# otiliastr/coper

Hardware: AMD Instinct MI355X
Metric: scored triples/sec (1-vs-all) (higher is better)
Workload: dtype fp16x3 (fp32 values split into two fp16 terms, 3 fp16 MFMAs per product, fp32 accumulate; comparisons closer than the split's error decided by the fp32 chain)

## Files before the change

### coper_amd/csrc/kernels_dense_fused_bf16.hip

```cpp
#include "bf16x3_chain.h"
#include "coper_internal.h"
#ifdef COPER_DBG_GROUP_CLK
#include <hip/hip_runtime.h>
__device__ unsigned long long g_group_clk[8];
extern "C" __attribute__((visibility("default"))) int coper_dbg_group_clock(unsigned long long* out) {
  return hipMemcpyFromSymbol(out, HIP_SYMBOL(g_group_clk), sizeof(unsigned long long) * 8) == hipSuccess ? 0 : 1;
}
#define GROUP_CLK(i) do { __syncthreads(); if (threadIdx.x == 0) g_group_clk[i] = wall_clock64(); } while (0)
#endif
#include "group_body.h"
#include "conv_fold.h"

namespace coper {

typedef float f32x4 __attribute__((ext_vector_type(4)));
typedef unsigned u32x4 __attribute__((ext_vector_type(4)));

#define MFMA16_BF16(a, b, c) S16_MFMA16(a, b, c)
#define MFMA16_X3(ahi, alo, bhi, blo, c) \
  { (c) = MFMA16_BF16(alo, bhi, c); (c) = MFMA16_BF16(ahi, blo, c); (c) = MFMA16_BF16(ahi, bhi, c); }


#ifndef COPER_FUSED_PMAX
#define COPER_FUSED_PMAX 3
#endif
#ifndef COPER_FUSED_PBUDGET
#define COPER_FUSED_PBUDGET 220
#endif


#define FW_DECL u32x4 W[P][NW][2]
#define FW_HI(s_, j_) W[s_][j_][0]
#define FW_LO(s_, j_) W[s_][j_][1]
#define FW_LO_RAW(s_, j_) W[s_][j_][1]
#define FW_PRE(s_)
#define FW_WREG3 (3 * NW * 8)

struct FusedConvArgs {
  const float* e1_rows;
  const int32_t* sorted_row;
  const int32_t* sorted_rid;
  const float* ent;
  const float* rel_emb;
  const float* conv_w;
  const float* conv_b;
  const float* scale;
  const float* shift;
  int per_rel_conv, d, r, in_w, in_hw, Wo, img_stride, x_exp;
  int img_exp;
  int64_t* chk;
  int w_div, w_rem;
  int32_t* bad;
};

#ifdef COPER_DBG_FUSED_CLOCK
__device__ unsigned long long g_fused_ph[8 * 2048];
extern "C" __attribute__((visibility("default"))) int coper_dbg_fused_phases(unsigned long long* out, int n) {
  return hipMemcpyFromSymbol(out, HIP_SYMBOL(g_fused_ph), sizeof(unsigned long long) * 8 * (n < 2048 ? n : 2048)) == hipSuccess ? 0 : 1;
}
#define FUSED_PH(i_)                                                                                            \
  do {                                                                                                          \
    const int w_ = blockIdx.x + gridDim.x * (blockIdx.y + gridDim.y * blockIdx.z);                              \
    if ((threadIdx.x & 63) == 0 && w_ < 2048) g_fused_ph[8 * w_ + (i_)] = __builtin_amdgcn_s_memrealtime();     \
  } while (0)
#else
#define FUSED_PH(i_) do { } while (0)
#endif
struct FusedFinConst {
  const int32_t* perm; const float* fc_b; const float* scale; const float* shift; const int32_t* w_exp; float* x3m;
  int per_rel_bias, x_exp, d, pad;
};
struct FusedFin {
  float* h_out; const FusedFinConst* c;
};
constexpr int FUSED_STAGE_WGS = 16;


__device__ __forceinline__ void fused_load_images(unsigned* __restrict__ img, const FusedConvArgs& A, int start, int n,
                                                  int t0, int t1) {
  const int wave = __builtin_amdgcn_readfirstlane(threadIdx.x >> 6), lane = threadIdx.x & 63;
  const int q0 = wave * 16;
  if (q0 < n) {
    int qi = q0 + (lane & 15);
    if (qi > n - 1) qi = n - 1;
    int my_row = A.sorted_row[start + qi], my_rid = A.sorted_rid[start + qi];
#ifdef COPER_DBG_NO_GROUP_CHK
    const bool chk = false;
#else
    const bool chk = A.chk != nullptr && (blockIdx.y | blockIdx.z) == 0;
#endif
    int64_t live_rel = 0, live_e1 = 0;
    const int chk_row = my_row, chk_rid = my_rid;
    if (chk) group_chk_issue(A.chk, start + qi, live_rel, live_e1);
#ifdef COPER_DBG_FUSED_NO_IMG
    my_row = -1;
#endif
    const float* base = A.e1_rows ? A.e1_rows : A.ent;
    const int len = t1 - t0, PD = (A.img_stride - 1) >> 1, eI = A.img_exp;
    auto fetch2 = [&](const int row, const int rid, const int t) -> float2 {
      if (t >= t1) return make_float2(0.f, 0.f);
      if (t < A.d) return row >= 0 ? *(const float2*)(base + (int64_t)row * A.d + t) : make_float2(0.f, 0.f);
      return *(const float2*)(A.rel_emb + (int64_t)rid * A.r + (t - A.d));
    };
    auto put2 = [&](const int q, const int pp, const float2 x) {
      unsigned short h0, l0, h1, l1;
      split1_s16(x3_scale(x.x, eI), h0, l0);
      split1_s16(x3_scale(x.y, eI), h1, l1);
      img[q * A.img_stride + pp] = (unsigned)h0 | ((unsigned)h1 << 16);
      img[q * A.img_stride + PD + pp] = (unsigned)l0 | ((unsigned)l1 << 16);
    };
    float2 v[16][2];
#pragma unroll
    for (int u = 0; u < 16; ++u) {
      const int row = __builtin_amdgcn_readlane(my_row, u), rid = __builtin_amdgcn_readlane(my_rid, u);
#pragma unroll
      for (int h = 0; h < 2; ++h) v[u][h] = fetch2(row, rid, t0 + 2 * (lane + 64 * h));
    }
#pragma unroll
    for (int u = 0; u < 16; ++u)
      if (q0 + u < n) {
#pragma unroll
        for (int h = 0; h < 2; ++h)
          if (2 * (lane + 64 * h) < len) put2(q0 + u, lane + 64 * h, v[u][h]);
        if (lane == 0) img[(q0 + u) * A.img_stride + 2 * PD] = 0u;
      }
    if (len > 256) {
      for (int u = 0; u < 16 && q0 + u < n; ++u) {
        const int row = __builtin_amdgcn_readlane(my_row, u), rid = __builtin_amdgcn_readlane(my_rid, u);
        for (int pp = 128 + lane; 2 * pp < len; pp += 64) put2(q0 + u, pp, fetch2(row, rid, t0 + 2 * pp));
      }
    }
    if (chk) group_chk_verdict(A.chk, live_rel, live_e1, chk_row, chk_rid);
  }
  asm volatile("s_waitcnt lgkmcnt(0)" ::: "memory");
  __builtin_amdgcn_s_barrier();
}

typedef unsigned fused_img_t;
template <int NFB, int NB, bool WNT>
__device__ __forceinline__ void fused_matrix_role(const uint4* __restrict__ xring, fused_img_t* __restrict__ img,
                                                  const uint4* __restrict__ Whi, const uint4* __restrict__ Wlo,
                                                  const FusedConvArgs& A, int64_t relw, int64_t relw_w, int start, int n, int fb0,
                                                  int nfb, int64_t ks32n, int64_t kb, int64_t ke, int t0, int t1,
                                                  float* __restrict__ zdst, int d_pad16, int wave, const FusedFin& Fn, int64_t ks32s) {
  constexpr int NFULL = NFB / 4;
  constexpr int REM = NFB % 4 ? 1 : 0;
  static_assert(NFB % 4 <= 1, "at most one left-over feature block");
  constexpr int NRQ = REM ? (NB + 3) / 4 : 0;
  constexpr int NW = NFULL + REM;
  constexpr int P = (COPER_FUSED_PMAX >= 3 && (NFULL * NB + NRQ) * 4 + FW_WREG3 + 44 <= COPER_FUSED_PBUDGET) ? 3 : 2;
  constexpr int XSTAGE = 2 * NB * 64;
  const int lane = threadIdx.x & 63;
  const int nk = (int)(ke - kb);
  const uint4* wp[NW][2];
#pragma unroll
  for (int j = 0; j < NW; ++j) {
    int fb = fb0 + (j < NFULL ? wave + 4 * j : 4 * NFULL);
    if (fb > nfb - 1) fb = nfb - 1;
    int64_t o = ((relw_w * nfb + fb) * ks32s + kb) * 64;
    wp[j][0] = Whi + o;
    wp[j][1] = (const uint4*)(Wlo + o);
  }
  FW_DECL;
#define FUSED_W_LOAD(p_) (WNT ? __builtin_nontemporal_load(p_) : *(p_))
#define W_ISSUE(s, kk)                                                                                 \
  {                                                                                                    \
    _Pragma("unroll") for (int j = 0; j < NW; ++j) {                                                   \
      FW_HI(s, j) = FUSED_W_LOAD((const u32x4*)(wp[j][0] + (int64_t)(kk)*64) + lane);                 \
      FW_LO_RAW(s, j) = FUSED_W_LOAD((const u32x4*)((const uint4*)wp[j][1] + (int64_t)(kk)*64) + lane); \
    }                                                                                                  \
  }
#pragma unroll
  for (int t = 0; t < P; ++t)
    if (t < nk) W_ISSUE(t, t);
  if (wave == 0) FUSED_PH(0);
  fused_load_images(img, A, start, n, t0, t1);
  if (wave == 0) FUSED_PH(1);
  f32x4 acc[NFULL][NB], accr[NRQ > 0 ? NRQ : 1];
#pragma unroll
  for (int j = 0; j < NFULL; ++j)
#pragma unroll
    for (int q = 0; q < NB; ++q) acc[j][q] = (f32x4){0.f, 0.f, 0.f, 0.f};
#pragma unroll
  for (int t = 0; t < NRQ; ++t) accr[t] = (f32x4){0.f, 0.f, 0.f, 0.f};
#ifdef COPER_DBG_FUSED_NO_MFMA
#define M_STEP(s2)                                                                                  \
  {                                                                                                 \
    __builtin_amdgcn_s_barrier();                                                                   \
    const uint4* xb = xring + ((s2)&1) * XSTAGE + lane;                                             \
    _Pragma("unroll") for (int j = 0; j < NW; ++j) {                                                \
      acc[0][0][0] += __uint_as_float(FW_HI((s2) % P, j)[0] ^ FW_LO_RAW((s2) % P, j)[1]);           \
      acc[0][0][1] += __uint_as_float(FW_HI((s2) % P, j)[2] ^ FW_LO_RAW((s2) % P, j)[0]);           \
    }                                                                                               \
    acc[0][0][2] += __uint_as_float(xb[0].x);                                                       \
  }
#else
#ifdef COPER_DBG_FUSED_NO_XREAD
#define M_LD(i_) make_uint4((unsigned)lane, (unsigned)(i_), 0x3c003c00u, 0x3c003c00u)
#else
#define M_LD(i_) xb[i_]
#endif
#ifndef COPER_FUSED_XPF
#define COPER_FUSED_XPF 2
#endif
#ifndef COPER_FUSED_XBUDGET
#define COPER_FUSED_XBUDGET 220
#endif
  constexpr int NV = NB + (NRQ > 0 ? 1 : 0);
  constexpr int XPF = (P == 3 && (NFULL * NB + NRQ) * 4 + FW_WREG3 + 44 > COPER_FUSED_XBUDGET) ? 1 : COPER_FUSED_XPF, XR = XPF + 1;
  const int qr = wave < NB ? wave : NB - 1;
#define M_LDV_H(v_) M_LD(((v_) < NB ? (v_) : qr) * 64)
#define M_LDV_L(v_) M_LD((NB + ((v_) < NB ? (v_) : qr)) * 64)
#define M_STEP(s2)                                                                                  \
  {                                                                                                 \
    FW_PRE((s2) % P)                                                                                \
    __builtin_amdgcn_s_barrier();                                                                   \
    const uint4* xb = xring + ((s2)&1) * XSTAGE + lane;                                             \
    uint4 bhq[XR], blq[XR];                                                                         \
    _Pragma("unroll") for (int v = 0; v < XPF && v < NV; ++v) { bhq[v] = M_LDV_H(v); blq[v] = M_LDV_L(v); } \
    __builtin_amdgcn_sched_group_barrier(0x100, 2 * (XPF < NV ? XPF : NV), 0);                      \
    _Pragma("unroll") for (int q = 0; q < NB; ++q) {                                                \
      if (q + XPF < NV) {                                                                           \
        bhq[(q + XPF) % XR] = M_LDV_H(q + XPF); blq[(q + XPF) % XR] = M_LDV_L(q + XPF);             \
        __builtin_amdgcn_sched_group_barrier(0x100, 2, 0);                                          \
      }                                                                                             \
      __builtin_amdgcn_sched_group_barrier(0x008, 3 * NFULL, 0);                                    \
      const uint4 bh = bhq[q % XR], bl = blq[q % XR];                                               \
      _Pragma("unroll") for (int j = 0; j < NFULL; ++j)                                             \
          acc[j][q] = MFMA16_BF16(FW_LO((s2) % P, j), bh, acc[j][q]);                               \
      _Pragma("unroll") for (int j = 0; j < NFULL; ++j)                                             \
          acc[j][q] = MFMA16_BF16(FW_HI((s2) % P, j), bl, acc[j][q]);                               \
      _Pragma("unroll") for (int j = 0; j < NFULL; ++j)                                             \
          acc[j][q] = MFMA16_BF16(FW_HI((s2) % P, j), bh, acc[j][q]);                               \
    }                                                                                               \
    _Pragma("unroll") for (int t = 0; t < NRQ; ++t) {                                               \
      const int q = wave + 4 * t < NB ? wave + 4 * t : NB - 1;  \
      uint4 bh, bl;                                                                                 \
      if (t == 0) { bh = bhq[NB % XR]; bl = blq[NB % XR]; }     \
      else { bh = M_LD(q * 64); bl = M_LD((NB + q) * 64); }                                         \
      accr[t] = MFMA16_BF16(FW_LO((s2) % P, NFULL), bh, accr[t]);                                   \
      accr[t] = MFMA16_BF16(FW_HI((s2) % P, NFULL), bl, accr[t]);                                   \
      accr[t] = MFMA16_BF16(FW_HI((s2) % P, NFULL), bh, accr[t]);                                   \
    }                                                                                               \
  }
#endif
  int k0 = 0;
  for (; k0 + 2 * P <= nk; k0 += 2 * P) {
#pragma unroll
    for (int s2 = 0; s2 < 2 * P; ++s2) {
      M_STEP(s2);
#ifndef COPER_DBG_FUSED_NO_W
      const int kn = k0 + s2 + P;
      W_ISSUE(s2 % P, kn < nk ? kn : 0);
#endif
    }
    if (k0 == 0 && wave == 0) FUSED_PH(2);
  }
#pragma unroll
  for (int s2 = 0; s2 < 2 * P - 1; ++s2) {
    if (k0 + s2 < nk) {
      M_STEP(s2);
#ifndef COPER_DBG_FUSED_NO_W
      if (k0 + s2 + P < nk) W_ISSUE(s2 % P, k0 + s2 + P);
#endif
    }
  }
#undef M_STEP
#undef W_ISSUE
  if (wave == 0) FUSED_PH(3);
#ifdef COPER_DBG_FUSED_NO_STORE
  if (acc[0][0][0] != 1.2345f) return;
#endif
  if (Fn.h_out) {
    const FusedFinConst Fc = *Fn.c;
    const int d = Fc.d;
    const int zexp = -((Fc.w_exp ? Fc.w_exp[Fc.per_rel_bias ? relw : 0] : 0) + Fc.x_exp);
    const float* bsrc = Fc.per_rel_bias ? Fc.fc_b + relw * d : Fc.fc_b;
    float m = 0.f;
    int qrow[NB];
#pragma unroll
    for (int q = 0; q < NB; ++q) {
      const int qi = q * 16 + (lane & 15);
      qrow[q] = qi < n ? Fc.perm[start + qi] : -1;
    }
    auto fin = [&](const f32x4& a, const int fb, const int q, const float4& b4, const float4& s4, const float4& t4) {
      const int k0 = fb * 16 + 4 * (lane >> 4);
      if (fb >= nfb || qrow[q] < 0 || k0 >= d) return;
      float z0 = 0.f, z1 = 0.f, z2 = 0.f, z3 = 0.f;
      z0 += a[0]; z1 += a[1]; z2 += a[2]; z3 += a[3];
      float4 v;
      v.x = fmaxf(fmaf(x3_scale(z0, zexp) + b4.x, s4.x, t4.x), 0.f);
      v.y = fmaxf(fmaf(x3_scale(z1, zexp) + b4.y, s4.y, t4.y), 0.f);
      v.z = fmaxf(fmaf(x3_scale(z2, zexp) + b4.z, s4.z, t4.z), 0.f);
      v.w = fmaxf(fmaf(x3_scale(z3, zexp) + b4.w, s4.w, t4.w), 0.f);
      m = fmaxf(m, fmaxf(fmaxf(v.x, v.y), fmaxf(v.z, v.w)));
      *(float4*)(Fn.h_out + (int64_t)qrow[q] * d + k0) = v;
    };
    auto quad = [&](const float* p, const int fb) -> float4 {
      const int k0 = fb * 16 + 4 * (lane >> 4);
      return (fb < nfb && k0 < d) ? *(const float4*)(p + k0) : make_float4(0.f, 0.f, 0.f, 0.f);
    };
#pragma unroll
    for (int j = 0; j < NFULL; ++j) {
      const int fb = fb0 + wave + 4 * j;
      const float4 b4 = quad(bsrc, fb), s4 = quad(Fc.scale, fb), t4 = quad(Fc.shift, fb);
#pragma unroll
      for (int q = 0; q < NB; ++q) fin(acc[j][q], fb, q, b4, s4, t4);
    }
    if (NRQ > 0) {
      const int fb = fb0 + 4 * NFULL;
      const float4 b4 = quad(bsrc, fb), s4 = quad(Fc.scale, fb), t4 = quad(Fc.shift, fb);
#pragma unroll
      for (int t = 0; t < NRQ; ++t) {
        const int q = wave + 4 * t;
        if (q < NB) {
          const int qi = q * 16 + (lane & 15);
          const int row = qi < n ? Fc.perm[start + qi] : -1;
          const int k0 = fb * 16 + 4 * (lane >> 4);
          if (fb < nfb && row >= 0 && k0 < d) {
            float z0 = 0.f, z1 = 0.f, z2 = 0.f, z3 = 0.f;
            z0 += accr[t][0]; z1 += accr[t][1]; z2 += accr[t][2]; z3 += accr[t][3];
            float4 v;
            v.x = fmaxf(fmaf(x3_scale(z0, zexp) + b4.x, s4.x, t4.x), 0.f);
            v.y = fmaxf(fmaf(x3_scale(z1, zexp) + b4.y, s4.y, t4.y), 0.f);
            v.z = fmaxf(fmaf(x3_scale(z2, zexp) + b4.z, s4.z, t4.z), 0.f);
            v.w = fmaxf(fmaf(x3_scale(z3, zexp) + b4.w, s4.w, t4.w), 0.f);
            m = fmaxf(m, fmaxf(fmaxf(v.x, v.y), fmaxf(v.z, v.w)));
            *(float4*)(Fn.h_out + (int64_t)row * d + k0) = v;
          }
        }
      }
    }
#pragma unroll
    for (int o = 32; o >= 1; o >>= 1) m = fmaxf(m, __shfl_xor(m, o));
    if (lane == 0 && m > 0.f)
      atomicMax((unsigned*)&Fc.x3m[(blockIdx.x + gridDim.x * blockIdx.z) & (X3M_SLOTS - 1)], __float_as_uint(m));
    return;
  }
#pragma unroll
  for (int j = 0; j < NFULL; ++j) {
    const int fb = fb0 + wave + 4 * j;
#pragma unroll
    for (int q = 0; q < NB; ++q) {
      const int qi = q * 16 + (lane & 15);
      if (fb < nfb && qi < n) {
        float* dst = zdst + (int64_t)(start + qi) * d_pad16 + fb * 16 + 4 * (lane >> 4);
        *(float4*)dst = make_float4(acc[j][q][0], acc[j][q][1], acc[j][q][2], acc[j][q][3]);
      }
    }
  }
#pragma unroll
  for (int t = 0; t < NRQ; ++t) {
    const int fb = fb0 + 4 * NFULL, q = wave + 4 * t;
    const int qi = q * 16 + (lane & 15);
    if (fb < nfb && q < NB && qi < n) {
      float* dst = zdst + (int64_t)(start + qi) * d_pad16 + fb * 16 + 4 * (lane >> 4);
      *(float4*)dst = make_float4(accr[t][0], accr[t][1], accr[t][2], accr[t][3]);
    }
  }
}

template <int NB>
__device__ __forceinline__ void fused_conv_role(uint4* __restrict__ xring, unsigned* __restrict__ img,
                                                const FusedConvArgs& A, int64_t relw, int start, int n, int64_t kb,
                                                int64_t ke, int i_lo, int t0, int t1, int cw) {
  constexpr int NFR = (NB + 3) / 4;
  constexpr int XSTAGE = 2 * NB * 64;
  const int lane = threadIdx.x & 63;
  const int nk = (int)(ke - kb);
  const int Wo = A.Wo, in_w = A.in_w, W2 = in_w >> 1;
  const int g = lane >> 4, m = lane & 15;
  const int PD = (A.img_stride - 1) >> 1;
  u32x4 aop[2];
  f32x4 cop[2];
  {
    const float* wsrc = A.per_rel_conv ? A.conv_w + relw * (int64_t)(9 * 32) : A.conv_w;
    const float* bsrc = A.per_rel_conv ? A.conv_b + relw * (int64_t)32 : A.conv_b;
    const int te = A.x_exp - A.img_exp;
#pragma unroll
    for (int u = 0; u < 2; ++u) {
      const int ch = 8 * (m >> 2) + 4 * u + (m & 3);
      const float sc = A.scale[ch];
      unsigned short th[9], tl[9];
#pragma unroll
      for (int k = 0; k < 9; ++k) split1_s16(x3_scale(wsrc[k * 32 + ch] * sc, te), th[k], tl[k]);
      unsigned short sl[8];
#pragma unroll
      for (int k = 0; k < 8; ++k) sl[k] = g == 2 ? tl[k] : th[k];
      if (g == 3) {
        sl[0] = th[8]; sl[1] = th[8]; sl[2] = tl[8];
#pragma unroll
        for (int k = 3; k < 8; ++k) sl[k] = 0;
      }
#pragma unroll
      for (int k = 0; k < 4; ++k) aop[u][k] = (unsigned)sl[2 * k] | ((unsigned)sl[2 * k + 1] << 16);
#pragma unroll
      for (int i = 0; i < 4; ++i) {
        const int c = 8 * g + 4 * u + i;
        cop[u][i] = x3_scale(fmaf(bsrc[c], A.scale[c], A.shift[c]), A.x_exp);
      }
    }
  }
  fused_load_images(img, A, start, n, t0, t1);
  if (cw == 0) FUSED_PH(5);
  int qown[NFR], qoth[NFR];
#pragma unroll
  for (int t = 0; t < NFR; ++t) {
    int qi = (cw + 4 * t) * 16 + m;
    if (qi > n - 1) qi = n - 1;
    qown[t] = qi * A.img_stride + (g == 1 ? PD : 0);
    qoth[t] = qi * A.img_stride + (g == 1 ? 0 : PD);
  }
  int poff = (int)(kb - (int64_t)i_lo * Wo);
  int cj = poff;
  for (int kk = 0; kk <= nk; ++kk) {
    if (kk > 0) {
      asm volatile("s_waitcnt lgkmcnt(0)" ::: "memory");
      __builtin_amdgcn_s_barrier();
    }
#ifdef COPER_DBG_FUSED_NO_CONV
    if (kk < 1) {
#else
    if (kk < nk) {
#endif
      const int pd = poff >> 1;
      const unsigned sh = (unsigned)(poff & 1) << 4;
#pragma unroll
      for (int t = 0; t < NFR; ++t) {
        if (cw + 4 * t < NB) {
          const unsigned* r = img + qown[t] + pd;
          const unsigned d00 = r[0], d01 = r[1], d10 = r[W2], d11 = r[W2 + 1], d20 = r[2 * W2], d21 = r[2 * W2 + 1];
          const unsigned o21 = img[qoth[t] + pd + 2 * W2 + 1];
          const unsigned a01 = __builtin_amdgcn_alignbit(d01, d00, sh), a2 = d01 >> sh;
          const unsigned b01 = __builtin_amdgcn_alignbit(d11, d10, sh), b2 = d11 >> sh;
          const unsigned c01 = __builtin_amdgcn_alignbit(d21, d20, sh), c2 = d21 >> sh;
          u32x4 bop;
          bop[0] = a01;
          bop[1] = __builtin_amdgcn_perm(b01, a2, 0x05040100u);
          bop[2] = __builtin_amdgcn_perm(b2, b01, 0x05040302u);
          bop[3] = c01;
          if (g == 3) {
            bop[0] = __builtin_amdgcn_perm(o21 >> sh, c2, 0x05040100u);
            bop[1] = c2 & 0xffffu;
          }
          const f32x4 y0 = MFMA16_BF16(aop[0], bop, cop[0]);
          const f32x4 y1 = MFMA16_BF16(aop[1], bop, cop[1]);
          float y[8];
#pragma unroll
          for (int i = 0; i < 4; ++i) {
            y[i] = __builtin_amdgcn_fmed3f(y0[i], 0.f, 65504.f);
            y[4 + i] = __builtin_amdgcn_fmed3f(y1[i], 0.f, 65504.f);
          }
          uint4 h4, l4;
          split8_pos_s16(y, h4, l4);
          uint4* dst = xring + (kk & 1) * XSTAGE + (cw + 4 * t) * 64 + lane;
          dst[0] = h4;
          dst[NB * 64] = l4;
        }
      }
      if (++cj == Wo) { cj = 0; poff += in_w - Wo + 1; } else { ++poff; }
    }
  }
}

#ifdef COPER_DBG_FUSED_CLOCK
__device__ unsigned long long g_fused_clk[3 * 2048];
extern "C" __attribute__((visibility("default"))) int coper_dbg_fused_clock(unsigned long long* out, int n) {
  return hipMemcpyFromSymbol(out, HIP_SYMBOL(g_fused_clk), sizeof(unsigned long long) * 3 * (n < 2048 ? n : 2048)) == hipSuccess ? 0 : 1;
}
#endif

template <int NFB, bool WNT>
__global__ __launch_bounds__(512) void k_dense_fused_bf16x3(const uint4* __restrict__ Whi, const uint4* __restrict__ Wlo,
                                                            FusedConvArgs A, const int32_t* __restrict__ tiles,
                                                            const int32_t* __restrict__ n_tiles, int64_t cap_small,
                                                            int nfb, int64_t ks32n, int nslices, int64_t Bcap,
                                                            int d_pad16, float* __restrict__ z_part, FusedFin Fn,
                                                            int n_special, const int32_t* __restrict__ stage_src, int64_t stage_n,
                                                            int64_t* __restrict__ stage_dst, int64_t ks32s, GroupJob J, int n_group,
                                                            const int32_t* __restrict__ post_src, int64_t post_n, int32_t* __restrict__ post_dst) {
  extern __shared__ uint4 fused_lds[];
  if ((int)blockIdx.x < n_special) {
    if (blockIdx.y | blockIdx.z) return;
    const int n_copy = n_special - n_group;
    if ((int)blockIdx.x >= n_copy) {
      GROUP_CLK(0);
      if (J.wait_for > 0) {
        if (threadIdx.x == 0) {
          for (int spin = 0; spin < (1 << 21) && __hip_atomic_load(J.ticket, __ATOMIC_RELAXED, __HIP_MEMORY_SCOPE_AGENT) < J.wait_for; ++spin)
            __builtin_amdgcn_s_sleep(16);
          (void)__hip_atomic_load(J.ticket, __ATOMIC_ACQUIRE, __HIP_MEMORY_SCOPE_AGENT);
          __hip_atomic_store(J.ticket, 0, __ATOMIC_RELAXED, __HIP_MEMORY_SCOPE_AGENT);
        }
        __syncthreads();
      }
      GROUP_CLK(1);
      group_role_body<512>(J, (int*)fused_lds);
      GROUP_CLK(5);
      return;
    }
    const int64_t nb = n_copy, b = (int64_t)blockIdx.x;
    if (post_n > 0) {
      const bool pvec = ((((uintptr_t)post_src) | ((uintptr_t)post_dst)) & 15) == 0;
      const int64_t p4 = pvec ? post_n / 4 : 0;
      for (int64_t i = b * 512 + threadIdx.x; i < p4; i += nb * 512) ((int4*)post_dst)[i] = ((const int4*)post_src)[i];
      for (int64_t i = 4 * p4 + b * 512 + threadIdx.x; i < post_n; i += nb * 512) post_dst[i] = post_src[i];
    }
    const bool vec = ((((uintptr_t)stage_src) | ((uintptr_t)stage_dst)) & 15) == 0;
    const int64_t n4 = vec ? stage_n / 4 : 0;
    auto copy4 = [&](int64_t lo, int64_t hi) {
      for (int64_t i = lo + b * 512 + threadIdx.x; i < hi; i += nb * 512) {
        const int4 v = ((const int4*)stage_src)[i];
        longlong2* o = (longlong2*)(stage_dst + 4 * i);
        o[0] = make_longlong2(v.x, v.y);
        o[1] = make_longlong2(v.z, v.w);
      }
    };
    const bool sig = n_group && J.wait_for > 0;
    int64_t f4 = sig ? (J.front + 3) / 4 : 0;
    if (f4 > n4 || f4 * 4 < J.front) f4 = 0;
    for (int64_t i = b * 512 + threadIdx.x; i < f4; i += nb * 512) {
      const int4 v = ((const int4*)stage_src)[i];
      int64_t* o = stage_dst + 4 * i;
      __hip_atomic_store(o + 0, (int64_t)v.x, __ATOMIC_RELAXED, __HIP_MEMORY_SCOPE_AGENT);
      __hip_atomic_store(o + 1, (int64_t)v.y, __ATOMIC_RELAXED, __HIP_MEMORY_SCOPE_AGENT);
      __hip_atomic_store(o + 2, (int64_t)v.z, __ATOMIC_RELAXED, __HIP_MEMORY_SCOPE_AGENT);
      __hip_atomic_store(o + 3, (int64_t)v.w, __ATOMIC_RELAXED, __HIP_MEMORY_SCOPE_AGENT);
    }
    if (sig && f4 == 0)
      for (int64_t i = b * 512 + threadIdx.x; i < J.front; i += nb * 512)
        __hip_atomic_store(stage_dst + i, (int64_t)stage_src[i], __ATOMIC_RELAXED, __HIP_MEMORY_SCOPE_AGENT);
    if (sig) {
      __syncthreads();
      if (threadIdx.x == 0) __hip_atomic_fetch_add(J.ticket, 1, __ATOMIC_RELEASE, __HIP_MEMORY_SCOPE_AGENT);
    }
    copy4(f4, n4);
    for (int64_t i = 4 * n4 + b * 512 + threadIdx.x; i < stage_n; i += nb * 512) stage_dst[i] = stage_src[i];
    return;
  }
  int tile = (int)blockIdx.x - n_special;
  const int32_t* tl;
  {
    const int nbig = n_tiles[1];
    if (tile < nbig) {
      tl = tiles + 4 * (cap_small + tile);
    } else {
      tile -= nbig;
      if (tile >= n_tiles[0]) return;
      tl = tiles + 4 * (int64_t)tile;
    }
  }
#ifdef COPER_DBG_FUSED_EXIT
  return;
#endif
  const int slice = blockIdx.y;
  const int fb0 = blockIdx.z * NFB;
  const int64_t relw = __builtin_amdgcn_readfirstlane(tl[0]);
  int64_t relw_w = relw;
  if (A.w_div > 1) {
    relw_w = (int)relw / A.w_div;
    if ((int)relw - (int)relw_w * A.w_div != A.w_rem && threadIdx.x == 0 && (blockIdx.y | blockIdx.z) == 0) atomicAdd(A.bad, (int)tl[2]);
  }
  const int start = __builtin_amdgcn_readfirstlane(tl[1]);
  const int n = __builtin_amdgcn_readfirstlane(tl[2]);
  const bool shared_w = __builtin_amdgcn_readfirstlane(tl[3]) != 0;
  const int64_t kb = ks32n * slice / nslices, ke = ks32n * (slice + 1) / nslices;
  float* zdst = z_part + (int64_t)slice * Bcap * d_pad16;
  const int nb = (n + 15) >> 4;
  const int wave = __builtin_amdgcn_readfirstlane(threadIdx.x >> 6);
#ifdef COPER_DBG_FUSED_CLOCK
  const unsigned long long dbg_t0 = __builtin_amdgcn_s_memrealtime();
#endif
  uint4* xring = fused_lds;
  unsigned* img = (unsigned*)(fused_lds + 2 * 16 * 64);
  const int i_lo = (int)(kb / A.Wo);
  const int t0 = i_lo * A.in_w;
  int t1 = ((int)((ke - 1) / A.Wo) + 3) * A.in_w;
  if (t1 > A.in_hw) t1 = A.in_hw;
#define TILE_WNT(x_) (x_)
#define BODY(NB_)                                                                                                      \
  if (wave < 4) {                                                                                                      \
    if (WNT && !shared_w)                                                                                              \
      fused_matrix_role<NFB, NB_, TILE_WNT(true)>(xring, img, Whi, Wlo, A, relw, relw_w, start, n, fb0, nfb, ks32n, kb, ke, t0, t1, zdst, \
                                                  d_pad16, wave, Fn, ks32s);                                           \
    else                                                                                                               \
      fused_matrix_role<NFB, NB_, TILE_WNT(false)>(xring, img, Whi, Wlo, A, relw, relw_w, start, n, fb0, nfb, ks32n, kb, ke, t0, t1, zdst, \
                                                   d_pad16, wave, Fn, ks32s);                                          \
  } else                                                                                                               \
    fused_conv_role<NB_>(xring, img, A, relw, start, n, kb, ke, i_lo, t0, t1, wave - 4);
  switch (nb) {
    case 1: BODY(1); break;
    case 2: BODY(2); break;
    case 3: BODY(3); break;
    case 4: BODY(4); break;
    case 5: BODY(5); break;
    case 6: BODY(6); break;
    case 7: BODY(7); break;
    default: BODY(8); break;
  }
#undef BODY
#ifdef COPER_DBG_FUSED_CLOCK
  if (threadIdx.x == 0) {
    const int w = blockIdx.x + gridDim.x * (blockIdx.y + gridDim.y * blockIdx.z);
    if (w < 2048) { g_fused_clk[3 * w] = (unsigned long long)n; g_fused_clk[3 * w + 1] = dbg_t0; g_fused_clk[3 * w + 2] = __builtin_amdgcn_s_memrealtime(); }
  }
#endif
}

static int fused_rows_max(const Dims& dm, int nslices) {
  int64_t ks32n = dm.F_pad / 32;
  int m = 0;
  for (int s = 0; s < nslices; ++s) {
    int64_t kb = ks32n * s / nslices, ke = ks32n * (s + 1) / nslices;
    if (ke <= kb) continue;
    int rows = (int)((ke - 1) / dm.Wo) - (int)(kb / dm.Wo) + 3;
    if (rows > m) m = rows;
  }
  return m;
}

bool dense_fused_supported(const coper_handle* h, int nslices) {
  const Dims& dm = h->dm;
  if (!(dm.fh == 3 && dm.fw == 3 && dm.C == 32) || dm.concat_rel) return false;
  if (dm.F != dm.F_pad || dm.F != (int64_t)dm.Ho * dm.Wo * 32) return false;
  if (dm.gen_conv && !dm.gen_fc) return false;
  if (!(dm.nfb == 13 || dm.nfb == 8 || dm.nfb == 16)) return false;
  if ((dm.in_w & 1) || (dm.d & 1) || (dm.stacked && (dm.r & 1))) return false;
  int stride = fused_rows_max(dm, nslices) * dm.in_w;
  stride |= 1;
  size_t lds = (size_t)2 * 16 * 64 * sizeof(uint4) + (size_t)128 * stride * sizeof(float);
  return lds <= 160 * 1024;
}

template <int NFB, bool WNT>
static void dense_fused_launch(coper_handle* h, PassCtx& ctx, const int64_t* e1, const int64_t* rel, const float* e1_rows, int64_t B,
                               int nslices, int zgroups, float* h_fin, hipStream_t s) {
  const Dims& dm = h->dm;
  const coper_handle::GroupSet& cur = h->grouping();
  FusedFin Fn;
  Fn.h_out = h_fin; Fn.c = (const FusedFinConst*)cur.fin.get();
  int64_t cap_small = (dm.gen_fc ? dm.R : 1) + 1;
  FusedConvArgs A;
  A.e1_rows = e1_rows; A.sorted_row = cur.sorted_row; A.sorted_rid = cur.sorted_rid;
  A.ent = h->lv.ent_emb->ptr;
  A.rel_emb = rel_emb_or_null(h);
  A.conv_w = conv_w(h);
  A.conv_b = conv_b(h);
  A.scale = h->conv_scale; A.shift = h->conv_shift; A.x_exp = h->x_exp; A.img_exp = h->img_exp;
  A.per_rel_conv = dm.gen_conv ? 1 : 0;
  A.d = dm.d; A.r = dm.r; A.in_w = dm.in_w; A.in_hw = dm.in_h * dm.in_w; A.Wo = dm.Wo;
  A.img_stride = (fused_rows_max(dm, nslices) * dm.in_w) | 1;
  A.chk = ctx.chk;
  A.w_div = h->w_div; A.w_rem = h->w_rem; A.bad = cur.rel_count + dm.R + 1;
  size_t lds = (size_t)2 * 16 * 64 * sizeof(uint4) + (size_t)128 * A.img_stride * sizeof(float);
  static uint64_t attr_done = 0;
  const uint64_t bit = 1ull << (h->cfg.device & 63);
  if (!(attr_done & bit)) {
    (void)hipFuncSetAttribute((const void*)k_dense_fused_bf16x3<NFB, WNT>, hipFuncAttributeMaxDynamicSharedMemorySize, 160 * 1024);
    attr_done |= bit;
  }
  const int n_tile_blocks = (int)(B / 128 + (cap_small - 1 < B ? cap_small - 1 : B) + 1);
  coper_handle::PassPipeline& pp = h->pipe;
  bool capturing = false;
  if (pp.stage.n > 0 || pp.post.n > 0 || ctx.gnext_ride) {
    hipStreamCaptureStatus cap = hipStreamCaptureStatusNone;
    if (hipStreamIsCapturing(s, &cap) != hipSuccess) { (void)hipGetLastError(); capturing = true; }
    else capturing = cap != hipStreamCaptureStatusNone;
  }
  const bool stage_now = pp.stage.n > 0 && !capturing;
  const bool post_now = pp.post.n > 0 && ctx.post_here && !capturing;
  GroupJob J = {};
  int n_group = 0;
  if (ctx.gnext_ride && !capturing) {
    const int64_t R = dm.gen_fc ? dm.R : 1;
    const int t = h->gcur == 1 ? 2 : 1;
    const coper_handle::GroupSet& g = h->gset[t];
    if (g.slab && pp.gnext.B <= h->ws_queries && group_role_lds_ints(R, 512) * sizeof(int) <= lds) {
      J.B = pp.gnext.B; J.R = R; J.R_all = dm.R; J.shard_lo = h->cfg.shard_lo; J.n_local = dm.n_local; J.cap_small = cap_small;
      J.count = g.rel_count; J.offset = g.rel_offset; J.tiles = g.tiles; J.n_tiles = g.n_tiles; J.perm = g.perm;
      J.sorted_row = g.sorted_row; J.sorted_rid = g.sorted_rid; J.inv_perm = g.inv_perm; J.x3m = g.x3m; J.x3m_slots = X3M_SLOTS;
      J.chk = g.chk;
      J.use_rel = dm.gen_fc ? 1 : 0; J.have_e1_rows = pp.gnext.rows;
      auto in_stage = [&](const int64_t* p) { return stage_now && p && p + J.B > pp.stage.dst && p < pp.stage.dst + pp.stage.n; };
      J.rel64 = pp.gnext.rel; J.e1_64 = pp.gnext.e1;
      J.ticket = h->group_done() + 1;
      J.wait_for = (in_stage(pp.gnext.rel) || in_stage(pp.gnext.e1)) ? FUSED_STAGE_WGS : 0;
      J.front = 0;
      if (in_stage(pp.gnext.rel)) J.front = (pp.gnext.rel + J.B) - pp.stage.dst;
      if (in_stage(pp.gnext.e1) && (pp.gnext.e1 + J.B) - pp.stage.dst > J.front) J.front = (pp.gnext.e1 + J.B) - pp.stage.dst;
      if (J.front > pp.stage.n) J.front = pp.stage.n;
      n_group = 1;
      pp.gdone.e1 = pp.gnext.e1; pp.gdone.rel = pp.gnext.rel; pp.gdone.B = pp.gnext.B; pp.gdone.rows = pp.gnext.rows;
      pp.gdone.done = true; pp.gdone.set = t;
    }
  }
  const int n_stage = (stage_now || post_now) ? FUSED_STAGE_WGS : 0;
  hipLaunchKernelGGL((k_dense_fused_bf16x3<NFB, WNT>), dim3((unsigned)(n_tile_blocks + n_group + n_stage), (unsigned)nslices, (unsigned)zgroups), dim3(512),
                     lds, s, (const uint4*)h->Wf16_hi, (const uint4*)h->Wf16_lo, A, cur.tiles, cur.n_tiles, cap_small, dm.nfb,
                     dm.F_pad / 32, nslices, h->ws_queries, dm.d_pad16, h->z_part, Fn, n_group + n_stage, pp.stage.src,
                     stage_now ? pp.stage.n : 0, pp.stage.dst, w16_ks_stride(dm), J, n_group, pp.post.src, post_now ? pp.post.n : 0, pp.post.dst);
  if (stage_now) pp.take_stage();
  if (post_now) pp.take_post();
}

int fused_fin_update(coper_handle* h, hipStream_t s) {
  const Dims& dm = h->dm;
  if (!h->enc_bf16 || !h->home.x3m || !h->home.perm) return COPER_OK;
  for (int i = 0; i < 3; ++i) {
    coper_handle::GroupSet& g = h->gset[i];
    if (i > 0 && !g.slab) continue;
    FusedFinConst c;
    c.perm = g.perm; c.fc_b = fc_b(h); c.scale = h->fc_scale; c.shift = h->fc_shift;
    c.w_exp = h->w_exp; c.x3m = g.x3m; c.per_rel_bias = dm.gen_fc ? 1 : 0; c.x_exp = h->x_exp; c.d = dm.d; c.pad = 0;
    int rc;
    if ((rc = g.fin.ensure(h, sizeof c, "fused finalize constants"))) return rc;
    COPER_HIP_TRY(h, hipMemcpyAsync(g.fin, &c, sizeof c, hipMemcpyHostToDevice, s));
    COPER_HIP_TRY(h, hipStreamSynchronize(s));
    g.fused_fin_perm = g.perm;
  }
  return COPER_OK;
}

bool dense_fused_finalizes(const coper_handle* h, int nslices, const float* h_out) {
  static const bool off = getenv("COPER_FUSED_NO_FINALIZE") != nullptr;
  const Dims& dm = h->dm;
  const float* fcb = fc_b(h);
  const coper_handle::GroupSet& g = h->grouping();
  return !off && h_out && nslices == 1 && g.x3m && g.fin && g.fused_fin_perm == g.perm && (dm.d & 3) == 0 &&
         ((((uintptr_t)h_out) | ((uintptr_t)fcb) | ((uintptr_t)h->fc_scale.get()) | ((uintptr_t)h->fc_shift.get())) & 15) == 0;
}

int launch_dense_fused_bf16(coper_handle* h, PassCtx& ctx, const int64_t* e1, const int64_t* rel, const float* e1_rows, int64_t B,
                            int nslices, float* h_fin, hipStream_t s) {
  if (!dense_fused_finalizes(h, nslices, h_fin)) h_fin = nullptr;
#ifndef COPER_FUSED_SPLIT_B
#define COPER_FUSED_SPLIT_B 2048
#endif
  const bool wnt = h->dm.gen_fc && B * 2 <= 128 * h->dm.R;
#define FUSED_GO(NFB_, Z_)                                                             \
  {                                                                                    \
    if (wnt) dense_fused_launch<NFB_, true>(h, ctx, e1, rel, e1_rows, B, nslices, Z_, h_fin, s);   \
    else dense_fused_launch<NFB_, false>(h, ctx, e1, rel, e1_rows, B, nslices, Z_, h_fin, s);      \
  }
  if (B <= COPER_FUSED_SPLIT_B / 2) FUSED_GO(4, (h->dm.nfb + 3) / 4)
  else if (h->dm.nfb == 13 && B > COPER_FUSED_SPLIT_B) FUSED_GO(13, 1)
  else FUSED_GO(8, (h->dm.nfb + 7) / 8)
#undef FUSED_GO
  COPER_HIP_TRY(h, hipGetLastError());
  return COPER_OK;
}

}
```

Baseline: 45.07 million.

## Move left-over feature block matmul from matrix waves to conv waves

The single left-over feature block (when NFB%4==1) is no longer computed by the four matrix waves, each of which carried an extra accumulator and weight stage. It is now computed by the conv waves, which keep their own deep weight prefetch ring and run the 3-MFMA split product on the x fragments they just produced, then apply the finishing epilogue themselves. Freeing those registers lets the matrix waves use a prefetch depth of up to 4 when the budget allows. The cost is more register pressure and MFMA work on the conv waves, which could lengthen their critical path and delay the barrier-synchronized x ring.

```diff
diff --git a/coper_amd/csrc/kernels_dense_fused_bf16.hip b/coper_amd/csrc/kernels_dense_fused_bf16.hip
--- a/coper_amd/csrc/kernels_dense_fused_bf16.hip
+++ b/coper_amd/csrc/kernels_dense_fused_bf16.hip
@@ -22,11 +22,18 @@
 
 
 #ifndef COPER_FUSED_PMAX
-#define COPER_FUSED_PMAX 3
+#define COPER_FUSED_PMAX 4
 #endif
 #ifndef COPER_FUSED_PBUDGET
 #define COPER_FUSED_PBUDGET 220
 #endif
+constexpr int fused_regs(int acc, int wstage, int p) { return acc + wstage * p + 44; }
+constexpr int fused_depth(int acc, int wstage, int pmax) {
+  int p = 2;
+  for (int t = 3; t <= pmax; ++t)
+    if (fused_regs(acc, wstage, t) <= COPER_FUSED_PBUDGET) p = t;
+  return p;
+}
 
 
 #define FW_DECL u32x4 W[P][NW][2]
@@ -34,7 +41,6 @@
 #define FW_LO(s_, j_) W[s_][j_][1]
 #define FW_LO_RAW(s_, j_) W[s_][j_][1]
 #define FW_PRE(s_)
-#define FW_WREG3 (3 * NW * 8)
 
 struct FusedConvArgs {
   const float* e1_rows;
@@ -75,6 +81,29 @@
 };
 constexpr int FUSED_STAGE_WGS = 16;
 
+#define FUSED_FIN_LAMBDAS                                                                                                      \
+    auto fin = [&](const f32x4& a, const int fb, const int q, const float4& b4, const float4& s4, const float4& t4) {           \
+      const int k0 = fb * 16 + 4 * (lane >> 4);                                                                                \
+      if (fb >= nfb || qrow[q] < 0 || k0 >= d) return;                                                                         \
+      float z0 = 0.f, z1 = 0.f, z2 = 0.f, z3 = 0.f;        \
+      z0 += a[0]; z1 += a[1]; z2 += a[2]; z3 += a[3];                                                                          \
+      float4 v;                                                                                                                \
+      v.x = fmaxf(fmaf(x3_scale(z0, zexp) + b4.x, s4.x, t4.x), 0.f);                                                           \
+      v.y = fmaxf(fmaf(x3_scale(z1, zexp) + b4.y, s4.y, t4.y), 0.f);                                                           \
+      v.z = fmaxf(fmaf(x3_scale(z2, zexp) + b4.z, s4.z, t4.z), 0.f);                                                           \
+      v.w = fmaxf(fmaf(x3_scale(z3, zexp) + b4.w, s4.w, t4.w), 0.f);                                                           \
+      m = fmaxf(m, fmaxf(fmaxf(v.x, v.y), fmaxf(v.z, v.w)));                                                                   \
+      *(float4*)(Fn.h_out + (int64_t)qrow[q] * d + k0) = v;                                                                    \
+    };                                                                                                                         \
+    auto quad = [&](const float* p, const int fb) -> float4 {                                                                  \
+      const int k0 = fb * 16 + 4 * (lane >> 4);                                                                                \
+      return (fb < nfb && k0 < d) ? *(const float4*)(p + k0) : make_float4(0.f, 0.f, 0.f, 0.f);                                \
+    };
+#define FUSED_FIN_MAX                                                                                                          \
+    _Pragma("unroll") for (int o = 32; o >= 1; o >>= 1) m = fmaxf(m, __shfl_xor(m, o));                                        \
+    if (lane == 0 && m > 0.f)                                                                                                  \
+      atomicMax((unsigned*)&Fc.x3m[(blockIdx.x + gridDim.x * blockIdx.z) & (X3M_SLOTS - 1)], __float_as_uint(m));
+
 
 __device__ __forceinline__ void fused_load_images(unsigned* __restrict__ img, const FusedConvArgs& A, int start, int n,
                                                   int t0, int t1) {
@@ -144,18 +173,19 @@
                                                   int nfb, int64_t ks32n, int64_t kb, int64_t ke, int t0, int t1,
                                                   float* __restrict__ zdst, int d_pad16, int wave, const FusedFin& Fn, int64_t ks32s) {
   constexpr int NFULL = NFB / 4;
-  constexpr int REM = NFB % 4 ? 1 : 0;
   static_assert(NFB % 4 <= 1, "at most one left-over feature block");
-  constexpr int NRQ = REM ? (NB + 3) / 4 : 0;
-  constexpr int NW = NFULL + REM;
-  constexpr int P = (COPER_FUSED_PMAX >= 3 && (NFULL * NB + NRQ) * 4 + FW_WREG3 + 44 <= COPER_FUSED_PBUDGET) ? 3 : 2;
+  constexpr int NW = NFULL;
+  constexpr int PCAP = (NFB % 4) ? COPER_FUSED_PMAX : (COPER_FUSED_PMAX < 3 ? COPER_FUSED_PMAX : 3);
+  constexpr int P = fused_depth(NFULL * NB * 4, 8 * NW, PCAP);
+  static_assert(P >= 2 && P <= 4, "prefetch depth");
+  static_assert(P == 2 || fused_regs(NFULL * NB * 4, 8 * NW, P) <= COPER_FUSED_PBUDGET, "the prefetch stages do not fit the register budget");
   constexpr int XSTAGE = 2 * NB * 64;
   const int lane = threadIdx.x & 63;
   const int nk = (int)(ke - kb);
   const uint4* wp[NW][2];
 #pragma unroll
   for (int j = 0; j < NW; ++j) {
-    int fb = fb0 + (j < NFULL ? wave + 4 * j : 4 * NFULL);
+    int fb = fb0 + wave + 4 * j;
     if (fb > nfb - 1) fb = nfb - 1;
     int64_t o = ((relw_w * nfb + fb) * ks32s + kb) * 64;
     wp[j][0] = Whi + o;
@@ -176,13 +206,11 @@
   if (wave == 0) FUSED_PH(0);
   fused_load_images(img, A, start, n, t0, t1);
   if (wave == 0) FUSED_PH(1);
-  f32x4 acc[NFULL][NB], accr[NRQ > 0 ? NRQ : 1];
+  f32x4 acc[NFULL][NB];
 #pragma unroll
   for (int j = 0; j < NFULL; ++j)
 #pragma unroll
     for (int q = 0; q < NB; ++q) acc[j][q] = (f32x4){0.f, 0.f, 0.f, 0.f};
-#pragma unroll
-  for (int t = 0; t < NRQ; ++t) accr[t] = (f32x4){0.f, 0.f, 0.f, 0.f};
 #ifdef COPER_DBG_FUSED_NO_MFMA
 #define M_STEP(s2)                                                                                  \
   {                                                                                                 \
@@ -206,11 +234,11 @@
 #ifndef COPER_FUSED_XBUDGET
 #define COPER_FUSED_XBUDGET 220
 #endif
-  constexpr int NV = NB + (NRQ > 0 ? 1 : 0);
-  constexpr int XPF = (P == 3 && (NFULL * NB + NRQ) * 4 + FW_WREG3 + 44 > COPER_FUSED_XBUDGET) ? 1 : COPER_FUSED_XPF, XR = XPF + 1;
-  const int qr = wave < NB ? wave : NB - 1;
-#define M_LDV_H(v_) M_LD(((v_) < NB ? (v_) : qr) * 64)
-#define M_LDV_L(v_) M_LD((NB + ((v_) < NB ? (v_) : qr)) * 64)
+  constexpr int NV = NB;
+  constexpr int XPF = (P >= 3 && fused_regs(NFULL * NB * 4, 8 * NW, P) > COPER_FUSED_XBUDGET) ? 1 : COPER_FUSED_XPF, XR = XPF + 1;
+  static_assert(COPER_FUSED_XBUDGET < COPER_FUSED_PBUDGET || XPF == COPER_FUSED_XPF, "a depth within the budget keeps the x fragments two blocks ahead");
+#define M_LDV_H(v_) M_LD((v_) * 64)
+#define M_LDV_L(v_) M_LD((NB + (v_)) * 64)
 #define M_STEP(s2)                                                                                  \
   {                                                                                                 \
     FW_PRE((s2) % P)                                                                                \
@@ -233,21 +261,13 @@
       _Pragma("unroll") for (int j = 0; j < NFULL; ++j)                                             \
           acc[j][q] = MFMA16_BF16(FW_HI((s2) % P, j), bh, acc[j][q]);                               \
     }                                                                                               \
-    _Pragma("unroll") for (int t = 0; t < NRQ; ++t) {                                               \
-      const int q = wave + 4 * t < NB ? wave + 4 * t : NB - 1;  \
-      uint4 bh, bl;                                                                                 \
-      if (t == 0) { bh = bhq[NB % XR]; bl = blq[NB % XR]; }     \
-      else { bh = M_LD(q * 64); bl = M_LD((NB + q) * 64); }                                         \
-      accr[t] = MFMA16_BF16(FW_LO((s2) % P, NFULL), bh, accr[t]);                                   \
-      accr[t] = MFMA16_BF16(FW_HI((s2) % P, NFULL), bl, accr[t]);                                   \
-      accr[t] = MFMA16_BF16(FW_HI((s2) % P, NFULL), bh, accr[t]);                                   \
-    }                                                                                               \
-  }
-#endif
+  }
+#endif
+  constexpr int U = (P & 1) ? 2 * P : P;
   int k0 = 0;
-  for (; k0 + 2 * P <= nk; k0 += 2 * P) {
-#pragma unroll
-    for (int s2 = 0; s2 < 2 * P; ++s2) {
+  for (; k0 + U <= nk; k0 += U) {
+#pragma unroll
+    for (int s2 = 0; s2 < U; ++s2) {
       M_STEP(s2);
 #ifndef COPER_DBG_FUSED_NO_W
       const int kn = k0 + s2 + P;
@@ -257,7 +277,7 @@
     if (k0 == 0 && wave == 0) FUSED_PH(2);
   }
 #pragma unroll
-  for (int s2 = 0; s2 < 2 * P - 1; ++s2) {
+  for (int s2 = 0; s2 < U - 1; ++s2) {
     if (k0 + s2 < nk) {
       M_STEP(s2);
 #ifndef COPER_DBG_FUSED_NO_W
@@ -283,23 +303,7 @@
       const int qi = q * 16 + (lane & 15);
       qrow[q] = qi < n ? Fc.perm[start + qi] : -1;
     }
-    auto fin = [&](const f32x4& a, const int fb, const int q, const float4& b4, const float4& s4, const float4& t4) {
-      const int k0 = fb * 16 + 4 * (lane >> 4);
-      if (fb >= nfb || qrow[q] < 0 || k0 >= d) return;
-      float z0 = 0.f, z1 = 0.f, z2 = 0.f, z3 = 0.f;
-      z0 += a[0]; z1 += a[1]; z2 += a[2]; z3 += a[3];
-      float4 v;
-      v.x = fmaxf(fmaf(x3_scale(z0, zexp) + b4.x, s4.x, t4.x), 0.f);
-      v.y = fmaxf(fmaf(x3_scale(z1, zexp) + b4.y, s4.y, t4.y), 0.f);
-      v.z = fmaxf(fmaf(x3_scale(z2, zexp) + b4.z, s4.z, t4.z), 0.f);
-      v.w = fmaxf(fmaf(x3_scale(z3, zexp) + b4.w, s4.w, t4.w), 0.f);
-      m = fmaxf(m, fmaxf(fmaxf(v.x, v.y), fmaxf(v.z, v.w)));
-      *(float4*)(Fn.h_out + (int64_t)qrow[q] * d + k0) = v;
-    };
-    auto quad = [&](const float* p, const int fb) -> float4 {
-      const int k0 = fb * 16 + 4 * (lane >> 4);
-      return (fb < nfb && k0 < d) ? *(const float4*)(p + k0) : make_float4(0.f, 0.f, 0.f, 0.f);
-    };
+    FUSED_FIN_LAMBDAS
 #pragma unroll
     for (int j = 0; j < NFULL; ++j) {
       const int fb = fb0 + wave + 4 * j;
@@ -307,34 +311,7 @@
 #pragma unroll
       for (int q = 0; q < NB; ++q) fin(acc[j][q], fb, q, b4, s4, t4);
     }
-    if (NRQ > 0) {
-      const int fb = fb0 + 4 * NFULL;
-      const float4 b4 = quad(bsrc, fb), s4 = quad(Fc.scale, fb), t4 = quad(Fc.shift, fb);
-#pragma unroll
-      for (int t = 0; t < NRQ; ++t) {
-        const int q = wave + 4 * t;
-        if (q < NB) {
-          const int qi = q * 16 + (lane & 15);
-          const int row = qi < n ? Fc.perm[start + qi] : -1;
-          const int k0 = fb * 16 + 4 * (lane >> 4);
-          if (fb < nfb && row >= 0 && k0 < d) {
-            float z0 = 0.f, z1 = 0.f, z2 = 0.f, z3 = 0.f;
-            z0 += accr[t][0]; z1 += accr[t][1]; z2 += accr[t][2]; z3 += accr[t][3];
-            float4 v;
-            v.x = fmaxf(fmaf(x3_scale(z0, zexp) + b4.x, s4.x, t4.x), 0.f);
-            v.y = fmaxf(fmaf(x3_scale(z1, zexp) + b4.y, s4.y, t4.y), 0.f);
-            v.z = fmaxf(fmaf(x3_scale(z2, zexp) + b4.z, s4.z, t4.z), 0.f);
-            v.w = fmaxf(fmaf(x3_scale(z3, zexp) + b4.w, s4.w, t4.w), 0.f);
-            m = fmaxf(m, fmaxf(fmaxf(v.x, v.y), fmaxf(v.z, v.w)));
-            *(float4*)(Fn.h_out + (int64_t)row * d + k0) = v;
-          }
-        }
-      }
-    }
-#pragma unroll
-    for (int o = 32; o >= 1; o >>= 1) m = fmaxf(m, __shfl_xor(m, o));
-    if (lane == 0 && m > 0.f)
-      atomicMax((unsigned*)&Fc.x3m[(blockIdx.x + gridDim.x * blockIdx.z) & (X3M_SLOTS - 1)], __float_as_uint(m));
+    FUSED_FIN_MAX
     return;
   }
 #pragma unroll
@@ -349,25 +326,42 @@
       }
     }
   }
-#pragma unroll
-  for (int t = 0; t < NRQ; ++t) {
-    const int fb = fb0 + 4 * NFULL, q = wave + 4 * t;
-    const int qi = q * 16 + (lane & 15);
-    if (fb < nfb && q < NB && qi < n) {
-      float* dst = zdst + (int64_t)(start + qi) * d_pad16 + fb * 16 + 4 * (lane >> 4);
-      *(float4*)dst = make_float4(accr[t][0], accr[t][1], accr[t][2], accr[t][3]);
-    }
-  }
-}
-
-template <int NB>
+}
+
+#ifndef COPER_FUSED_PR
+#define COPER_FUSED_PR 6
+#endif
+template <int NFB, int NB, bool WNT>
 __device__ __forceinline__ void fused_conv_role(uint4* __restrict__ xring, unsigned* __restrict__ img,
-                                                const FusedConvArgs& A, int64_t relw, int start, int n, int64_t kb,
-                                                int64_t ke, int i_lo, int t0, int t1, int cw) {
+                                                const uint4* __restrict__ Whi, const uint4* __restrict__ Wlo,
+                                                const FusedConvArgs& A, int64_t relw, int64_t relw_w, int start, int n, int fb0,
+                                                int nfb, int64_t kb, int64_t ke, int i_lo, int t0, int t1,
+                                                float* __restrict__ zdst, int d_pad16, int cw, const FusedFin& Fn, int64_t ks32s) {
   constexpr int NFR = (NB + 3) / 4;
   constexpr int XSTAGE = 2 * NB * 64;
+  constexpr bool DENSE = NFB % 4 == 1;
+  constexpr int PR = COPER_FUSED_PR;
+  static_assert(PR >= 4 && 8 * PR + 12 * NFR + 100 <= COPER_FUSED_PBUDGET, "the conv role's prefetch stages do not fit the register budget");
   const int lane = threadIdx.x & 63;
   const int nk = (int)(ke - kb);
+  const uint4 *wph = nullptr, *wpl = nullptr;
+  u32x4 WR[PR][2];
+#define CW_LOAD(p_) (WNT ? __builtin_nontemporal_load(p_) : *(p_))
+#define CW_ISSUE(s, kk)                                                              \
+  {                                                                                  \
+    WR[s][0] = CW_LOAD((const u32x4*)(wph + (int64_t)(kk)*64) + lane);               \
+    WR[s][1] = CW_LOAD((const u32x4*)(wpl + (int64_t)(kk)*64) + lane);               \
+  }
+  if constexpr (DENSE) {
+    int fb = fb0 + 4 * (NFB / 4);
+    if (fb > nfb - 1) fb = nfb - 1;
+    const int64_t o = ((relw_w * nfb + fb) * ks32s + kb) * 64;
+    wph = Whi + o;
+    wpl = Wlo + o;
+#pragma unroll
+    for (int t = 0; t < PR; ++t)
+      if (t < nk) CW_ISSUE(t, t);
+  }
   const int Wo = A.Wo, in_w = A.in_w, W2 = in_w >> 1;
   const int g = lane >> 4, m = lane & 15;
   const int PD = (A.img_stride - 1) >> 1;
@@ -413,54 +407,178 @@
   }
   int poff = (int)(kb - (int64_t)i_lo * Wo);
   int cj = poff;
-  for (int kk = 0; kk <= nk; ++kk) {
-    if (kk > 0) {
-      asm volatile("s_waitcnt lgkmcnt(0)" ::: "memory");
-      __builtin_amdgcn_s_barrier();
-    }
+#define CONV_X(t_, kk_, H_, L_)                                                                                    \
+  {                                                                                                                \
+    const unsigned* r = img + qown[t_] + pd;                                                                       \
+    const unsigned d00 = r[0], d01 = r[1], d10 = r[W2], d11 = r[W2 + 1], d20 = r[2 * W2], d21 = r[2 * W2 + 1];     \
+    const unsigned o21 = img[qoth[t_] + pd + 2 * W2 + 1];                                                          \
+    const unsigned a01 = __builtin_amdgcn_alignbit(d01, d00, sh), a2 = d01 >> sh;                                  \
+    const unsigned b01 = __builtin_amdgcn_alignbit(d11, d10, sh), b2 = d11 >> sh;                                  \
+    const unsigned c01 = __builtin_amdgcn_alignbit(d21, d20, sh), c2 = d21 >> sh;                                  \
+    u32x4 bop;                                                                                                     \
+    bop[0] = a01;                                                                                   \
+    bop[1] = __builtin_amdgcn_perm(b01, a2, 0x05040100u);                                           \
+    bop[2] = __builtin_amdgcn_perm(b2, b01, 0x05040302u);                                           \
+    bop[3] = c01;                                                                                   \
+    if (g == 3) {                                                   \
+      bop[0] = __builtin_amdgcn_perm(o21 >> sh, c2, 0x05040100u);                                                  \
+      bop[1] = c2 & 0xffffu;                                                                                       \
+    }                                                                                                              \
+    const f32x4 y0 = MFMA16_BF16(aop[0], bop, cop[0]);                                                             \
+    const f32x4 y1 = MFMA16_BF16(aop[1], bop, cop[1]);                                                             \
+    float y[8];                                                                                                    \
+    _Pragma("unroll") for (int i = 0; i < 4; ++i) {                                                                \
+      y[i] = __builtin_amdgcn_fmed3f(y0[i], 0.f, 65504.f);                                                         \
+      y[4 + i] = __builtin_amdgcn_fmed3f(y1[i], 0.f, 65504.f);                                                     \
+    }                                                                                                              \
+    split8_pos_s16(y, H_, L_);                                                                                     \
+    uint4* dst = xring + ((kk_) & 1) * XSTAGE + (cw + 4 * (t_)) * 64 + lane;                                       \
+    dst[0] = H_;                                                                                                   \
+    dst[NB * 64] = L_;                                                                                             \
+  }
+#define CONV_NEXT if (++cj == Wo) { cj = 0; poff += in_w - Wo + 1; } else { ++poff; }
+  if constexpr (!DENSE) {
+    for (int kk = 0; kk <= nk; ++kk) {
+      if (kk > 0) {
+        asm volatile("s_waitcnt lgkmcnt(0)" ::: "memory");
+        __builtin_amdgcn_s_barrier();
+      }
 #ifdef COPER_DBG_FUSED_NO_CONV
-    if (kk < 1) {
+      if (kk < 1) {
 #else
-    if (kk < nk) {
-#endif
-      const int pd = poff >> 1;
-      const unsigned sh = (unsigned)(poff & 1) << 4;
+      if (kk < nk) {
+#endif
+        const int pd = poff >> 1;
+        const unsigned sh = (unsigned)(poff & 1) << 4;
+#pragma unroll
+        for (int t = 0; t < NFR; ++t) {
+          if (cw + 4 * t < NB) {
+            uint4 h4, l4;
+            CONV_X(t, kk, h4, l4);
+          }
+        }
+        CONV_NEXT
+      }
+    }
+  } else {
+    uint4 xh[NFR], xl[NFR];
+    f32x4 accd[NFR];
+#pragma unroll
+    for (int t = 0; t < NFR; ++t) {
+      xh[t] = xl[t] = make_uint4(0u, 0u, 0u, 0u);
+      accd[t] = (f32x4){0.f, 0.f, 0.f, 0.f};
+    }
+#ifdef COPER_DBG_FUSED_NO_MFMA
+#define CW_DENSE(s_)                                                                                   \
+  {                                                                                                    \
+    accd[0][0] += __uint_as_float(WR[s_][0][0] ^ WR[s_][1][1]);                                        \
+    accd[0][1] += __uint_as_float(WR[s_][0][2] ^ WR[s_][1][0] ^ xh[0].x);                              \
+  }
+#else
+#define CW_DENSE(s_)                                                                                   \
+  {                                                                                                    \
+    _Pragma("unroll") for (int t = 0; t < NFR; ++t) accd[t] = MFMA16_BF16(WR[s_][1], xh[t], accd[t]);  \
+    _Pragma("unroll") for (int t = 0; t < NFR; ++t) accd[t] = MFMA16_BF16(WR[s_][0], xl[t], accd[t]);  \
+    _Pragma("unroll") for (int t = 0; t < NFR; ++t) accd[t] = MFMA16_BF16(WR[s_][0], xh[t], accd[t]);  \
+  }
+#endif
+#define CW_CONV(kk_, h_, l_)                                                                           \
+  {                                                                                                    \
+    const int pd = poff >> 1;                                                                          \
+    const unsigned sh = (unsigned)(poff & 1) << 4;                                                     \
+    _Pragma("unroll") for (int t = 0; t < NFR; ++t)                                                    \
+      if (cw + 4 * t < NB) CONV_X(t, kk_, h_[t], l_[t])        \
+    CONV_NEXT                                                                                          \
+  }
+#ifdef COPER_DBG_FUSED_NO_CONV
+#define CW_CONV_K(kk_, h_, l_) { }
+#else
+#define CW_CONV_K(kk_, h_, l_) CW_CONV(kk_, h_, l_)
+#endif
+#ifdef COPER_FUSED_DENSE_LAST
+#define CW_STEP(s_, k_, last_)                                                                         \
+  {                                                                                                    \
+    asm volatile("s_waitcnt lgkmcnt(0)" ::: "memory");   \
+    __builtin_amdgcn_s_barrier();                                                                      \
+    uint4 nh[NFR], nl[NFR];                                                                            \
+    _Pragma("unroll") for (int t = 0; t < NFR; ++t) { nh[t] = xh[t]; nl[t] = xl[t]; }                  \
+    if (!(last_)) CW_CONV_K((k_) + 1, nh, nl);                                                         \
+    CW_DENSE(s_);                                                                                      \
+    _Pragma("unroll") for (int t = 0; t < NFR; ++t) { xh[t] = nh[t]; xl[t] = nl[t]; }                  \
+  }
+#else
+#define CW_STEP(s_, k_, last_)                                                                         \
+  {                                                                                                    \
+    asm volatile("s_waitcnt lgkmcnt(0)" ::: "memory");   \
+    __builtin_amdgcn_s_barrier();                                                                      \
+    CW_DENSE(s_);                                                                                      \
+    if (!(last_)) CW_CONV_K((k_) + 1, xh, xl);                                                         \
+  }
+#endif
+    CW_CONV(0, xh, xl);
+    if (cw == 0) FUSED_PH(6);
+    constexpr int U = (PR & 1) ? 2 * PR : PR;
+    int k0 = 0;
+    for (; k0 + U < nk; k0 += U) {
+#pragma unroll
+      for (int s2 = 0; s2 < U; ++s2) {
+        CW_STEP(s2 % PR, k0 + s2, false);
+#ifndef COPER_DBG_FUSED_NO_W
+        const int kn = k0 + s2 + PR;
+        CW_ISSUE(s2 % PR, kn < nk ? kn : 0);
+#endif
+      }
+    }
+#pragma unroll
+    for (int s2 = 0; s2 < U; ++s2) {
+      if (k0 + s2 < nk) {
+        CW_STEP(s2 % PR, k0 + s2, k0 + s2 + 1 >= nk);
+#ifndef COPER_DBG_FUSED_NO_W
+        if (k0 + s2 + PR < nk) CW_ISSUE(s2 % PR, k0 + s2 + PR);
+#endif
+      }
+    }
+    if (cw == 0) FUSED_PH(7);
+#undef CW_STEP
+#undef CW_CONV_K
+#undef CW_CONV
+#undef CW_DENSE
+#ifdef COPER_DBG_FUSED_NO_STORE
+    if (accd[0][0] != 1.2345f) return;
+#endif
+    const int fb = fb0 + 4 * (NFB / 4);
+    if (Fn.h_out) {
+      const FusedFinConst Fc = *Fn.c;
+      const int d = Fc.d;
+      const int zexp = -((Fc.w_exp ? Fc.w_exp[Fc.per_rel_bias ? relw : 0] : 0) + Fc.x_exp);
+      const float* bsrc = Fc.per_rel_bias ? Fc.fc_b + relw * d : Fc.fc_b;
+      float m = 0.f;
+      int qrow[NFR];
 #pragma unroll
       for (int t = 0; t < NFR; ++t) {
-        if (cw + 4 * t < NB) {
-          const unsigned* r = img + qown[t] + pd;
-          const unsigned d00 = r[0], d01 = r[1], d10 = r[W2], d11 = r[W2 + 1], d20 = r[2 * W2], d21 = r[2 * W2 + 1];
-          const unsigned o21 = img[qoth[t] + pd + 2 * W2 + 1];
-          const unsigned a01 = __builtin_amdgcn_alignbit(d01, d00, sh), a2 = d01 >> sh;
-          const unsigned b01 = __builtin_amdgcn_alignbit(d11, d10, sh), b2 = d11 >> sh;
-          const unsigned c01 = __builtin_amdgcn_alignbit(d21, d20, sh), c2 = d21 >> sh;
-          u32x4 bop;
-          bop[0] = a01;
-          bop[1] = __builtin_amdgcn_perm(b01, a2, 0x05040100u);
-          bop[2] = __builtin_amdgcn_perm(b2, b01, 0x05040302u);
-          bop[3] = c01;
-          if (g == 3) {
-            bop[0] = __builtin_amdgcn_perm(o21 >> sh, c2, 0x05040100u);
-            bop[1] = c2 & 0xffffu;
-          }
-          const f32x4 y0 = MFMA16_BF16(aop[0], bop, cop[0]);
-          const f32x4 y1 = MFMA16_BF16(aop[1], bop, cop[1]);
-          float y[8];
-#pragma unroll
-          for (int i = 0; i < 4; ++i) {
-            y[i] = __builtin_amdgcn_fmed3f(y0[i], 0.f, 65504.f);
-            y[4 + i] = __builtin_amdgcn_fmed3f(y1[i], 0.f, 65504.f);
-          }
-          uint4 h4, l4;
-          split8_pos_s16(y, h4, l4);
-          uint4* dst = xring + (kk & 1) * XSTAGE + (cw + 4 * t) * 64 + lane;
-          dst[0] = h4;
-          dst[NB * 64] = l4;
-        }
-      }
-      if (++cj == Wo) { cj = 0; poff += in_w - Wo + 1; } else { ++poff; }
-    }
-  }
+        const int qi = (cw + 4 * t) * 16 + (lane & 15);
+        qrow[t] = (cw + 4 * t < NB && qi < n) ? Fc.perm[start + qi] : -1;
+      }
+      FUSED_FIN_LAMBDAS
+      const float4 b4 = quad(bsrc, fb), s4 = quad(Fc.scale, fb), t4 = quad(Fc.shift, fb);
+#pragma unroll
+      for (int t = 0; t < NFR; ++t) fin(accd[t], fb, t, b4, s4, t4);
+      FUSED_FIN_MAX
+      return;
+    }
+#pragma unroll
+    for (int t = 0; t < NFR; ++t) {
+      const int qi = (cw + 4 * t) * 16 + (lane & 15);
+      if (fb < nfb && cw + 4 * t < NB && qi < n) {
+        float* dst = zdst + (int64_t)(start + qi) * d_pad16 + fb * 16 + 4 * (lane >> 4);
+        *(float4*)dst = make_float4(accd[t][0], accd[t][1], accd[t][2], accd[t][3]);
+      }
+    }
+  }
+#undef CW_ISSUE
+#undef CW_LOAD
+#undef CONV_NEXT
+#undef CONV_X
 }
 
 #ifdef COPER_DBG_FUSED_CLOCK
@@ -587,7 +705,14 @@
       fused_matrix_role<NFB, NB_, TILE_WNT(false)>(xring, img, Whi, Wlo, A, relw, relw_w, start, n, fb0, nfb, ks32n, kb, ke, t0, t1, zdst, \
                                                    d_pad16, wave, Fn, ks32s);                                          \
   } else                                                                                                               \
-    fused_conv_role<NB_>(xring, img, A, relw, start, n, kb, ke, i_lo, t0, t1, wave - 4);
+  {                                                                                                             \
+    if (NFB % 4 == 1 && WNT && !shared_w)        \
+      fused_conv_role<NFB, NB_, TILE_WNT(true)>(xring, img, Whi, Wlo, A, relw, relw_w, start, n, fb0, nfb, kb, ke, i_lo, t0, t1, zdst, \
+                                                d_pad16, wave - 4, Fn, ks32s);                                         \
+    else                                                                                                               \
+      fused_conv_role<NFB, NB_, TILE_WNT(false)>(xring, img, Whi, Wlo, A, relw, relw_w, start, n, fb0, nfb, kb, ke, i_lo, t0, t1, zdst, \
+                                                 d_pad16, wave - 4, Fn, ks32s);                                        \
+  }
   switch (nb) {
     case 1: BODY(1); break;
     case 2: BODY(2); break;
```

Result: no change. 45.19 million (median of 2 runs) (+0.3%).
